# Pasqui1010/DART-Planner

Hardware: AMD Instinct MI355X
Metric: SE(3) rollouts/sec (N=30, batch=8192) + p95 solve ms, at 1/2/4/8 MI355X (higher is better)
Workload: dtype f32

## Files before the change

### dart_planner_amd/csrc/closed_loop_device.hpp

```cpp
#pragma once
#include <hip/hip_runtime.h>

#include <cmath>

#include "se3mpc_common.hpp"

static_assert(sizeof(se3mpc_controller_params) == 304, "se3mpc_controller_params is part of the C ABI (capi.py mirrors it)");
static_assert(sizeof(se3mpc_simulator_params) == 56, "se3mpc_simulator_params is part of the C ABI");

namespace se3mpc {

template <typename R>
struct CtrlDev {
  R kp_pos[3], ki_pos[3], kd_pos[3], kp_att[3], kd_att[3], inertia[3], max_torque[3], max_int_axis[3];
  R max_integral_pos, max_tilt, cos_max_tilt, gravity, max_thrust, min_thrust_abs, hover, track_thr, vel_thr, kb, decay, sat_thr,
      yaw_sing_thr, dh_cos, dh_sin;
  int anti_windup, fallback;
};

template <typename R>
static CtrlDev<R> make_ctrl_dev(const se3mpc_controller_params& p) {
  CtrlDev<R> c;
  for (int i = 0; i < 3; ++i) {
    c.kp_pos[i] = (R)p.kp_pos[i]; c.ki_pos[i] = (R)p.ki_pos[i]; c.kd_pos[i] = (R)p.kd_pos[i];
    c.kp_att[i] = (R)p.kp_att[i]; c.kd_att[i] = (R)p.kd_att[i]; c.inertia[i] = (R)p.inertia[i];
    c.max_torque[i] = (R)p.max_torque_xyz[i]; c.max_int_axis[i] = (R)p.max_integral_per_axis[i];
  }
  c.max_integral_pos = (R)p.max_integral_pos; c.max_tilt = (R)p.max_tilt_angle; c.cos_max_tilt = (R)std::cos(p.max_tilt_angle);
  c.gravity = (R)p.gravity; c.max_thrust = (R)p.max_thrust;
  c.min_thrust_abs = (R)(p.min_thrust * p.mass * p.gravity);
  c.hover = (R)(p.mass * p.gravity);
  c.track_thr = (R)p.tracking_error_threshold; c.vel_thr = (R)p.velocity_error_threshold;
  c.kb = (R)p.back_calculation_gain; c.decay = (R)p.integral_decay_factor; c.sat_thr = (R)p.saturation_threshold;
  c.yaw_sing_thr = (R)p.yaw_singularity_threshold;
  c.dh_cos = (R)std::cos(p.default_heading_yaw); c.dh_sin = (R)std::sin(p.default_heading_yaw);
  c.anti_windup = p.anti_windup_method; c.fallback = p.yaw_fallback_method;
  return c;
}

template <typename R>
struct SimDev {
  R mass, gravity, inertia[3], max_thrust, max_torque;
};
template <typename R>
static SimDev<R> make_sim_dev(const se3mpc_simulator_params& p) {
  SimDev<R> s;
  s.mass = (R)p.mass; s.gravity = (R)p.gravity; s.max_thrust = (R)p.max_thrust; s.max_torque = (R)p.max_torque;
  for (int i = 0; i < 3; ++i) s.inertia[i] = (R)p.inertia[i];
  return s;
}

template <typename R>
struct CtrlRegs {
  R integral[3];
  double last_time;
  R last_valid_thrust, unsat_thrust, unsat_torque[3];
  int failsafe_count, halvings, flags;
};

template <typename R>
__device__ __forceinline__ CtrlRegs<R> load_ctrl(const double* __restrict__ s) {
  CtrlRegs<R> r;
  for (int i = 0; i < 3; ++i) { r.integral[i] = (R)s[i]; r.unsat_torque[i] = (R)s[6 + i]; }
  r.last_time = s[3]; r.last_valid_thrust = (R)s[4]; r.unsat_thrust = (R)s[5];
  r.failsafe_count = (int)s[9]; r.halvings = (int)s[10]; r.flags = (int)s[11];
  return r;
}
template <typename R>
__device__ __forceinline__ void store_ctrl(double* __restrict__ s, const CtrlRegs<R>& r) {
  for (int i = 0; i < 3; ++i) { s[i] = (double)r.integral[i]; s[6 + i] = (double)r.unsat_torque[i]; }
  s[3] = r.last_time; s[4] = (double)r.last_valid_thrust; s[5] = (double)r.unsat_thrust;
  s[9] = (double)r.failsafe_count; s[10] = (double)r.halvings; s[11] = (double)r.flags;
}

template <typename R>
__device__ __forceinline__ R norm3(const R v[3]) { return sqrt(v[0] * v[0] + v[1] * v[1] + v[2] * v[2]); }
__device__ __forceinline__ void sin_cos(float x, float& s, float& c) { sincosf(x, &s, &c); }
__device__ __forceinline__ void sin_cos(double x, double& s, double& c) { sincos(x, &s, &c); }
template <typename R>
__device__ __forceinline__ R sign_of(R v) { return v > (R)0 ? (R)1 : (v < (R)0 ? (R)-1 : v); }
template <typename R>
__device__ __forceinline__ void cross3(const R a[3], const R b[3], R o[3]) {
  o[0] = a[1] * b[2] - a[2] * b[1]; o[1] = a[2] * b[0] - a[0] * b[2]; o[2] = a[0] * b[1] - a[1] * b[0];
}

template <typename R>
__device__ __forceinline__ void enter_failsafe(CtrlRegs<R>& s) {
  if (!(s.flags & 1)) {
    s.halvings += 1;
    s.integral[0] = s.integral[1] = s.integral[2] = (R)0;
    s.failsafe_count += 1;
  }
  s.flags |= 1;
}

enum { CF_FAILSAFE = 1, CF_BAD_DT = 2, CF_THRUST_SAT = 4, CF_SINGULAR = 8, CF_TILT = 16, CF_TORQUE_SAT_X = 32 };

template <typename R>
__device__ __forceinline__ void update_integral(const CtrlDev<R>& c, CtrlRegs<R>& s, const R ve[3], R dt, bool thrust_sat) {
  R upd[3];
  for (int i = 0; i < 3; ++i) upd[i] = ve[i] * dt;
  if (c.anti_windup == 0) {
    if (thrust_sat) for (int i = 0; i < 3; ++i) upd[i] = upd[i] * (R)0.1;
    for (int i = 0; i < 3; ++i) if (s.flags & (4 << i)) upd[i] = upd[i] * (R)0.1;
  } else if (c.anti_windup == 1) {
    if (thrust_sat) {
      const R fb = (s.unsat_thrust - c.max_thrust) * c.kb;
      upd[0] = upd[0] - fb * (R)0.33; upd[1] = upd[1] - fb * (R)0.33; upd[2] = upd[2] - fb * (R)0.34;
    }
    for (int i = 0; i < 3; ++i)
      if (s.flags & (4 << i)) upd[i] = upd[i] - ((s.unsat_torque[i] - c.max_torque[i]) * c.kb) * (R)0.5;
  }
  R I[3];
  for (int i = 0; i < 3; ++i) {
    I[i] = s.integral[i] + upd[i];
    if (fabs(I[i]) > c.max_int_axis[i]) I[i] = sign_of(I[i]) * c.max_int_axis[i];
  }
  const R mag = norm3(I);
  if (mag > c.max_integral_pos) { const R f = c.max_integral_pos / mag; for (int i = 0; i < 3; ++i) I[i] = I[i] * f; }
  for (int i = 0; i < 3; ++i) {
    if (fabs(I[i]) > c.max_int_axis[i] * c.sat_thr) I[i] = I[i] * c.decay;
    s.integral[i] = I[i];
  }
}

template <typename R>
__device__ __forceinline__ void desired_frame(const CtrlDev<R>& c, int method, bool force, const R yv[3], const R b3n[3], R cy, R sy, R b1[3],
                                              R b2[3], R& cos_angle, bool& singular) {
  cos_angle = fabs((yv[0] * b3n[0] + yv[1] * b3n[1]) + yv[2] * b3n[2]);
  singular = cos_angle >= c.yaw_sing_thr;
  if (singular || force) {
    R proj[3] = {(R)1 - b3n[0] * b3n[0], (R)0 - b3n[0] * b3n[1], (R)0 - b3n[0] * b3n[2]};
    const R np_ = norm3(proj);
    proj[0] = proj[0] / np_; proj[1] = proj[1] / np_; proj[2] = proj[2] / np_;
    if (method == 1 || method == 2) {
      const R hv[3] = {method == 1 ? c.dh_cos : cy, method == 1 ? c.dh_sin : sy, (R)0};
      R cx[3];
      cross3(hv, b3n, cx);
      const R nc = norm3(cx);
      if (nc > (R)1e-6) { b1[0] = cx[0] / nc; b1[1] = cx[1] / nc; b1[2] = cx[2] / nc; }
      else { b1[0] = proj[0]; b1[1] = proj[1]; b1[2] = proj[2]; }
    } else if (method != 0 || fabs(b3n[2]) < (R)0.99) {
      b1[0] = proj[0]; b1[1] = proj[1]; b1[2] = proj[2];
    } else {
      b1[0] = (R)1; b1[1] = (R)0; b1[2] = (R)0;
    }
  } else {
    cross3(yv, b3n, b1);
    const R n1 = norm3(b1);
    if (n1 > (R)1e-6) { b1[0] = b1[0] / n1; b1[1] = b1[1] / n1; b1[2] = b1[2] / n1; }
    else { b1[0] = (R)1; b1[1] = (R)0; b1[2] = (R)0; }
  }
  cross3(b3n, b1, b2);
}

template <typename R>
__device__ void attitude_torque(const CtrlDev<R>& c, CtrlRegs<R>& s, R scale, const R b3[3], const R att[3], const R omega[3], R yaw_des,
                                R yaw_rate_des, const R* Ifull, R torque_out[3], int& out_flags) {
  R cr, sr, cp, sp, cy, sy;
  sin_cos(att[0], sr, cr); sin_cos(att[1], sp, cp); sin_cos(att[2], sy, cy);
  const R Rm[3][3] = {{cy * cp, cy * sp * sr - sy * cr, cy * sp * cr + sy * sr},
                      {sy * cp, sy * sp * sr + cy * cr, sy * sp * cr - cy * sr},
                      {-sp, cp * sr, cp * cr}};
  R yc, ys;
  sin_cos(yaw_des, ys, yc);
  const R yv[3] = {yc, ys, (R)0};
  const R n3 = norm3(b3);
  const R b3n[3] = {b3[0] / n3, b3[1] / n3, b3[2] / n3};
  R b1[3], b2[3], cos_angle;
  bool singular;
  desired_frame(c, c.fallback, false, yv, b3n, cy, sy, b1, b2, cos_angle, singular);
  if (singular) out_flags |= CF_SINGULAR;
  const R Rd[3][3] = {{b1[0], b2[0], b3n[0]}, {b1[1], b2[1], b3n[1]}, {b1[2], b2[2], b3n[2]}};
  auto dtr = [&](const R A_[3][3], const R B_[3][3], int i, int j) { return (A_[0][i] * B_[0][j] + A_[1][i] * B_[1][j]) + A_[2][i] * B_[2][j]; };
  const R eR[3] = {(R)0.5 * (dtr(Rd, Rm, 2, 1) - dtr(Rm, Rd, 2, 1)), (R)0.5 * (dtr(Rd, Rm, 0, 2) - dtr(Rm, Rd, 0, 2)),
                   (R)0.5 * (dtr(Rd, Rm, 1, 0) - dtr(Rm, Rd, 1, 0))};
  const R eO[3] = {omega[0], omega[1], omega[2] - yaw_rate_des};
  R Iw[3];
  if (Ifull != nullptr) for (int i = 0; i < 3; ++i) Iw[i] = (Ifull[3 * i] * omega[0] + Ifull[3 * i + 1] * omega[1]) + Ifull[3 * i + 2] * omega[2];
  else for (int i = 0; i < 3; ++i) Iw[i] = c.inertia[i] * omega[i];
  R cor[3];
  cross3(omega, Iw, cor);
  int tsat = 0;
  for (int i = 0; i < 3; ++i) {
    R tq = (-(c.kp_att[i] * scale) * eR[i] - (c.kd_att[i] * scale) * eO[i]) + cor[i];
    s.unsat_torque[i] = tq;
    if (fabs(tq) > c.max_torque[i]) { tq = sign_of(tq) * c.max_torque[i]; tsat |= (4 << i); }
    torque_out[i] = tq;
  }
  s.flags = (s.flags & ~(4 | 8 | 16)) | tsat;
  out_flags |= (tsat >> 2) * CF_TORQUE_SAT_X;
}

template <typename R>
__device__ void attitude_command(const CtrlDev<R>& c, CtrlRegs<R>& s, R scale, const R tvw[3], R tm, const R att[3], const R omega[3],
                                 R yaw_des, R yaw_rate_des, R torque_out[3], int& out_flags) {
  R b3[3];
  if (tm > (R)1e-6) { b3[0] = tvw[0] / tm; b3[1] = tvw[1] / tm; b3[2] = tvw[2] / tm; }
  else { b3[0] = (R)0; b3[1] = (R)0; b3[2] = (R)1; }
  if (fmin(fmax(b3[2], (R)-1), (R)1) < c.cos_max_tilt) {
    const R sf = c.cos_max_tilt / b3[2];
    b3[0] = b3[0] * sf; b3[1] = b3[1] * sf; b3[2] = c.cos_max_tilt;
    const R n = norm3(b3);
    b3[0] = b3[0] / n; b3[1] = b3[1] / n; b3[2] = b3[2] / n;
    out_flags |= CF_TILT;
  }
  attitude_torque(c, s, scale, b3, att, omega, yaw_des, yaw_rate_des, (const R*)nullptr, torque_out, out_flags);
}

template <typename R>
__device__ void control_step(const CtrlDev<R>& c, CtrlRegs<R>& s, double t, const R pos[3], const R vel[3], const R att[3],
                             const R omega[3], const R dpos[3], const R dvel[3], const R dacc[3], R yaw_des, R yaw_rate_des,
                             R& thrust_out, R torque_out[3], int& out_flags) {
  out_flags = 0;
  const double dt_d = (s.last_time != s.last_time) ? 0.001 : t - s.last_time;
  s.last_time = t;
  if (dt_d <= 0.0 || dt_d > 0.1) {
    enter_failsafe(s);
    thrust_out = s.last_valid_thrust; torque_out[0] = torque_out[1] = torque_out[2] = (R)0;
    out_flags = CF_FAILSAFE | CF_BAD_DT;
    return;
  }
  const R dt = (R)dt_d;
  const R scale = (R)ldexp(1.0, -s.halvings);
  R pe[3], ve[3], tvw[3];
  for (int i = 0; i < 3; ++i) { pe[i] = dpos[i] - pos[i]; ve[i] = dvel[i] - vel[i]; }
  const R pen = norm3(pe), ven = norm3(ve);
  for (int i = 0; i < 3; ++i) {
    const R acc_pid = ((c.kp_pos[i] * scale) * pe[i] + (c.kd_pos[i] * scale) * ve[i]) + c.ki_pos[i] * s.integral[i];
    tvw[i] = dacc[i] + acc_pid;
  }
  tvw[2] = tvw[2] + c.gravity;
  R tm = norm3(tvw);
  s.unsat_thrust = tm;
  bool thrust_sat = false;
  if (tm > c.max_thrust) { tm = c.max_thrust; thrust_sat = true; }
  else if (tm < c.min_thrust_abs) { tm = c.min_thrust_abs; thrust_sat = true; }
  s.flags = (s.flags & ~2) | (thrust_sat ? 2 : 0);
  if (thrust_sat) out_flags |= CF_THRUST_SAT;
  update_integral(c, s, ve, dt, thrust_sat);
  if (pen > c.track_thr && ven > c.vel_thr) s.failsafe_count += 1;
  else s.failsafe_count = s.failsafe_count > 1 ? s.failsafe_count - 1 : 0;
  if (s.failsafe_count > 100) {
    enter_failsafe(s);
    thrust_out = s.last_valid_thrust; torque_out[0] = torque_out[1] = torque_out[2] = (R)0;
    out_flags |= CF_FAILSAFE;
    return;
  }
  attitude_command(c, s, scale, tvw, tm, att, omega, yaw_des, yaw_rate_des, torque_out, out_flags);
  s.last_valid_thrust = tm;
  s.flags &= ~1;
  s.failsafe_count = 0;
  thrust_out = tm;
}

template <typename R>
struct FastDev {
  R gravity, min_thrust_abs, hover;
};
template <typename R>
__device__ void control_step_fast(const CtrlDev<R>& c, const FastDev<R>& f, CtrlRegs<R>& s, double dt_d, const R pos[3], const R vel[3],
                                  const R att[3], const R omega[3], const R dpos[3], const R dvel[3], const R dacc[3], R yaw_des,
                                  R yaw_rate_des, R& thrust_out, R torque_out[3], int& out_flags) {
  out_flags = 0;
  if (dt_d <= 0.0 || dt_d > 0.1) {
    thrust_out = f.hover; torque_out[0] = torque_out[1] = torque_out[2] = (R)0;
    out_flags = CF_BAD_DT;
    return;
  }
  const R dt = (R)dt_d;
  const R scale = (R)ldexp(1.0, -s.halvings);
  R pe[3], ve[3], tvw[3];
  for (int i = 0; i < 3; ++i) { pe[i] = dpos[i] - pos[i]; ve[i] = dvel[i] - vel[i]; }
  for (int i = 0; i < 3; ++i) {
    const R acc_pid = ((c.kp_pos[i] * scale) * pe[i] + (c.kd_pos[i] * scale) * ve[i]) + c.ki_pos[i] * s.integral[i];
    tvw[i] = dacc[i] + acc_pid;
  }
  tvw[2] = tvw[2] + f.gravity;
  R tm = norm3(tvw);
  s.unsat_thrust = tm;
  bool thrust_sat = false;
  if (tm > c.max_thrust) { tm = c.max_thrust; thrust_sat = true; }
  else if (tm < f.min_thrust_abs) { tm = f.min_thrust_abs; thrust_sat = true; }
  s.flags = (s.flags & ~2) | (thrust_sat ? 2 : 0);
  if (thrust_sat) out_flags |= CF_THRUST_SAT;
  update_integral(c, s, ve, dt, thrust_sat);
  attitude_command(c, s, scale, tvw, tm, att, omega, yaw_des, yaw_rate_des, torque_out, out_flags);
  thrust_out = tm;
}

template <typename R>
struct PlanCursor {
  int idx;
  int rows_of;
  double t1, t2;
  R r1[9], r2[9];
};
template <typename R>
__device__ __forceinline__ void cursor_reset(PlanCursor<R>& c) { c.idx = 0; c.rows_of = -1; }

template <typename R>
__device__ __forceinline__ void sample_plan(double t, int N, const double* __restrict__ ts, const R* __restrict__ P, const R* __restrict__ V,
                                            const R* __restrict__ A, R tp[3], R tv[3], R ta[3], PlanCursor<R>& c) {
  int idx = c.idx;
  while (idx < N && ts[idx] < t) ++idx;
  c.idx = idx;
  if (idx != c.rows_of) {
    const int i1 = idx == 0 ? 0 : (idx >= N ? N - 1 : idx - 1), i2 = idx >= N ? N - 1 : idx;
    c.t1 = ts[i1]; c.t2 = ts[i2];
    for (int a = 0; a < 3; ++a) {
      c.r1[a] = P[3 * i1 + a]; c.r2[a] = P[3 * i2 + a];
      c.r1[3 + a] = V != nullptr ? V[3 * i1 + a] : (R)0; c.r2[3 + a] = V != nullptr ? V[3 * i2 + a] : (R)0;
      c.r1[6 + a] = A != nullptr ? A[3 * i1 + a] : (R)0; c.r2[6 + a] = A != nullptr ? A[3 * i2 + a] : (R)0;
    }
    c.rows_of = idx;
  }
  if (idx == 0 || idx >= N) {
    for (int a = 0; a < 3; ++a) { tp[a] = c.r1[a]; tv[a] = c.r1[3 + a]; ta[a] = c.r1[6 + a]; }
    return;
  }
  const R f = (R)((t - c.t1) / (c.t2 - c.t1));
  for (int a = 0; a < 3; ++a) {
    tp[a] = c.r1[a] + f * (c.r2[a] - c.r1[a]);
    tv[a] = c.r1[3 + a] + f * (c.r2[3 + a] - c.r1[3 + a]);
    ta[a] = c.r1[6 + a] + f * (c.r2[6 + a] - c.r1[6 + a]);
  }
}

template <typename R>
struct PlanView {
  int N;
  const double* ts; long long ts_stride;
  const R* P; long long sP;
  const R* V; long long sV;
  const R* A; long long sA;
  __device__ __forceinline__ PlanView of(int b) const {
    return {N, ts != nullptr ? ts + (size_t)b * ts_stride : nullptr, 0, P != nullptr ? P + (size_t)b * sP : nullptr, 0,
            V != nullptr ? V + (size_t)b * sV : nullptr, 0, A != nullptr ? A + (size_t)b * sA : nullptr, 0};
  }
};

template <typename R>
static inline bool plan_shape_ok(const PlanView<R>& p, int min_rows) {
  return p.N >= min_rows && p.N <= 4096 && p.ts_stride >= 0 && p.sP >= 0 && p.sV >= 0 && p.sA >= 0;
}
template <typename R>
static inline bool plan_present(const PlanView<R>& p) { return p.N <= 0 || (p.ts != nullptr && p.P != nullptr); }

template <typename R>
__device__ __forceinline__ void simulator_step(const SimDev<R>& m, R pos[3], R vel[3], R att[3], R omega[3], double& t, R thrust,
                                               const R torque[3], R dt, double dt_d, const R wind[3]) {
  thrust = fmin(fmax(thrust, (R)0), m.max_thrust);
  for (int i = 0; i < 3; ++i) {
    const R tq = fmin(fmax(torque[i], -m.max_torque), m.max_torque);
    const R wind_accel = wind[i] / m.mass;
    const R acc = ((i == 2 ? -m.gravity : (R)0) + (i == 2 ? thrust / m.mass : (R)0)) + wind_accel;
    vel[i] = vel[i] + acc * dt;
    pos[i] = pos[i] + vel[i] * dt;
    const R ang_acc = tq / m.inertia[i];
    omega[i] = omega[i] + ang_acc * dt;
    att[i] = att[i] + omega[i] * dt;
  }
  t = t + dt_d;
}

template <typename R>
__device__ __forceinline__ void cursor_before_step(PlanCursor<R>& cur, double sim_dt) {
  if (!(sim_dt > 0.0)) cur.idx = 0;
}

template <typename R>
__device__ __forceinline__ void flight_command(const CtrlDev<R>& c, CtrlRegs<R>& s, PlanCursor<R>& cur, int N, const double* ts, const R* P,
                                               const R* V, const R* A, const R p[3], const R v[3], const R a[3], const R w[3], double t,
                                               double sim_dt, R& th, R tq[3], R* target_row) {
  R tg[9];
  cursor_before_step(cur, sim_dt);
  sample_plan<R>(t, N, ts, P, V, A, tg, tg + 3, tg + 6, cur);
  if (target_row != nullptr) for (int i = 0; i < 9; ++i) target_row[i] = tg[i];
  int fl;
  control_step<R>(c, s, t, p, v, a, w, tg, tg + 3, tg + 6, (R)0, (R)0, th, tq, fl);
}

template <typename R>
__device__ __forceinline__ void flight_step(const CtrlDev<R>& c, const SimDev<R>& m, CtrlRegs<R>& s, PlanCursor<R>& cur, int N,
                                            const double* ts, const R* P, const R* V, const R* A, R p[3], R v[3], R a[3], R w[3], double& t,
                                            R dt, double sim_dt, const R wd[3], R& th, R tq[3]) {
  flight_command<R>(c, s, cur, N, ts, P, V, A, p, v, a, w, t, sim_dt, th, tq, (R*)nullptr);
  simulator_step<R>(m, p, v, a, w, t, th, tq, dt, sim_dt, wd);
}

template <typename R>
struct DroneBlock {
  double* stamps;
  double* time;
  double* ctrl;
  R *planP, *planV, *planA;
  R* vec;
};
template <typename R>
__device__ __forceinline__ DroneBlock<R> drone_block(unsigned char* base, int n, size_t plan_off, size_t vec_off) {
  DroneBlock<R> d;
  d.stamps = reinterpret_cast<double*>(base);
  d.time = d.stamps + n;
  d.ctrl = d.time + 1;
  d.planP = reinterpret_cast<R*>(base + plan_off);
  d.planV = d.planP + 3 * n;
  d.planA = d.planV + 3 * n;
  d.vec = reinterpret_cast<R*>(base + vec_off);
  return d;
}

template <typename R>
__device__ __forceinline__ void drone_load(const DroneBlock<R>& d, int b, const R* __restrict__ posg, const R* __restrict__ velg,
                                           const R* __restrict__ attg, const R* __restrict__ omegag, const R* __restrict__ windg,
                                           long long wind_stride, const double* __restrict__ timeg, const double* __restrict__ stateg) {
  for (int i = 0; i < 3; ++i) {
    d.vec[i] = posg[3 * b + i]; d.vec[3 + i] = velg[3 * b + i]; d.vec[6 + i] = attg[3 * b + i]; d.vec[9 + i] = omegag[3 * b + i];
    d.vec[12 + i] = windg != nullptr ? windg[(size_t)b * wind_stride + i] : (R)0;
  }
  *d.time = timeg[b];
  for (int i = 0; i < SE3MPC_CONTROLLER_STATE_WORDS; ++i) d.ctrl[i] = stateg[(size_t)b * SE3MPC_CONTROLLER_STATE_WORDS + i];
}
template <typename R>
__device__ __forceinline__ void drone_store(const DroneBlock<R>& d, int b, R* __restrict__ posg, R* __restrict__ velg, R* __restrict__ attg,
                                            R* __restrict__ omegag, double* __restrict__ timeg, double* __restrict__ stateg) {
  for (int i = 0; i < 3; ++i) { posg[3 * b + i] = d.vec[i]; velg[3 * b + i] = d.vec[3 + i]; attg[3 * b + i] = d.vec[6 + i]; omegag[3 * b + i] = d.vec[9 + i]; }
  timeg[b] = *d.time;
  for (int i = 0; i < SE3MPC_CONTROLLER_STATE_WORDS; ++i) stateg[(size_t)b * SE3MPC_CONTROLLER_STATE_WORDS + i] = d.ctrl[i];
}

template <typename IO>
__host__ __device__ constexpr size_t mc_plan_offset(int G) { return (size_t)(G + 1 + SE3MPC_CONTROLLER_STATE_WORDS) * sizeof(double); }
template <typename IO>
__host__ __device__ constexpr size_t mc_consts_offset(int G) { return (mc_plan_offset<IO>(G) + (size_t)(9 * G + 16) * sizeof(IO) + 15) / 16 * 16; }
template <typename IO>
__host__ __device__ constexpr size_t mc_group_bytes(int G) { return mc_consts_offset<IO>(G) + (sizeof(CtrlDev<IO>) + sizeof(SimDev<IO>) + 15) / 16 * 16; }

template <typename IO>
struct McBlock {
  DroneBlock<IO> d;
  CtrlDev<IO>* ctl;
  SimDev<IO>* sim;
};
template <typename IO, int G>
__device__ __forceinline__ McBlock<IO> mc_block(unsigned char* lds_raw, size_t solver_lds, int grp) {
  unsigned char* gb = lds_raw + solver_lds + (size_t)grp * mc_group_bytes<IO>(G);
  McBlock<IO> b;
  b.d = drone_block<IO>(gb, G, mc_plan_offset<IO>(G), mc_plan_offset<IO>(G) + (size_t)9 * G * sizeof(IO));
  b.ctl = reinterpret_cast<CtrlDev<IO>*>(gb + mc_consts_offset<IO>(G));
  b.sim = reinterpret_cast<SimDev<IO>*>(b.ctl + 1);
  return b;
}

#ifndef SE3MPC_MC_WAVES
#define SE3MPC_MC_WAVES 1
#endif

template <typename R>
struct DroneRegs {
  R p[3], v[3], a[3], w[3], wd[3];
  double t;
  __device__ __forceinline__ void load_state(int b, const R* __restrict__ pos, const R* __restrict__ vel, const R* __restrict__ att,
                                             const R* __restrict__ omega) {
    for (int i = 0; i < 3; ++i) { p[i] = pos[3 * b + i]; v[i] = vel[3 * b + i]; a[i] = att[3 * b + i]; w[i] = omega[3 * b + i]; }
  }
  __device__ __forceinline__ void load(int b, const R* __restrict__ pos, const R* __restrict__ vel, const R* __restrict__ att,
                                       const R* __restrict__ omega, const R* __restrict__ wind, long long wind_stride,
                                       const double* __restrict__ time) {
    load_state(b, pos, vel, att, omega);
    for (int i = 0; i < 3; ++i) wd[i] = wind != nullptr ? wind[(size_t)b * wind_stride + i] : (R)0;
    t = time[b];
  }
  __device__ __forceinline__ void store(int b, R* __restrict__ pos, R* __restrict__ vel, R* __restrict__ att, R* __restrict__ omega,
                                        double* __restrict__ time) const {
    for (int i = 0; i < 3; ++i) { pos[3 * b + i] = p[i]; vel[3 * b + i] = v[i]; att[3 * b + i] = a[i]; omega[3 * b + i] = w[i]; }
    time[b] = t;
  }
  __device__ __forceinline__ void load(const DroneBlock<R>& d) {
    for (int i = 0; i < 3; ++i) { p[i] = d.vec[i]; v[i] = d.vec[3 + i]; a[i] = d.vec[6 + i]; w[i] = d.vec[9 + i]; wd[i] = d.vec[12 + i]; }
    t = *d.time;
  }
  __device__ __forceinline__ void store(const DroneBlock<R>& d) const {
    for (int i = 0; i < 3; ++i) { d.vec[i] = p[i]; d.vec[3 + i] = v[i]; d.vec[6 + i] = a[i]; d.vec[9 + i] = w[i]; }
    *d.time = t;
  }
};

template <typename R, typename F>
__device__ __forceinline__ void fly_steps(const CtrlDev<R> c, const SimDev<R> m, const DroneBlock<R>& d, int N, int n, double sim_dt,
                                          F&& after_step) {
  CtrlRegs<R> s = load_ctrl<R>(d.ctrl);
  DroneRegs<R> r;
  r.load(d);
  const R dt = (R)sim_dt;
  PlanCursor<R> cur;
  cursor_reset(cur);
  for (int step = 0; step < n; ++step) {
    R th, tq[3];
    flight_step<R>(c, m, s, cur, N, d.stamps, d.planP, d.planV, d.planA, r.p, r.v, r.a, r.w, r.t, dt, sim_dt, r.wd, th, tq);
    after_step(step, r.p);
  }
  r.store(d);
  store_ctrl<R>(d.ctrl, s);
}

template <typename R, typename F>
__device__ __forceinline__ int lane_loop(DroneRegs<R>& d, int b, int B, int nsteps, int gust_step, R gx, R gy, R gz, bool stop_at_plan_end,
                                         double ts_last, R* __restrict__ log_state, R* __restrict__ log_cmd, double* __restrict__ log_time,
                                         F&& fly) {
  int taken = 0;
  bool active = true;
  for (int step = 0; step < nsteps; ++step) {
    if (stop_at_plan_end && d.t > ts_last) active = false;
    if (log_state != nullptr) {
      R* ls = log_state + ((size_t)step * B + b) * 12;
      for (int i = 0; i < 3; ++i) { ls[i] = d.p[i]; ls[3 + i] = d.v[i]; ls[6 + i] = d.a[i]; ls[9 + i] = d.w[i]; }
    }
    if (log_time != nullptr) log_time[(size_t)step * B + b] = d.t;
    R th = (R)NAN, tq[3] = {(R)NAN, (R)NAN, (R)NAN};
    if (active) {
      if (step == gust_step) { d.wd[0] = gx; d.wd[1] = gy; d.wd[2] = gz; }
      fly(step, th, tq);
      ++taken;
    }
    if (log_cmd != nullptr) {
      R* lc = log_cmd + ((size_t)step * B + b) * 4;
      lc[0] = th; lc[1] = tq[0]; lc[2] = tq[1]; lc[3] = tq[2];
    }
  }
  return taken;
}

static inline int check_controller_params(const se3mpc_controller_params* p) {
  if (p == nullptr) return SE3MPC_ERR_NULL;
  const double* d = reinterpret_cast<const double*>(p);
  for (int i = 0; i < 37; ++i)
    if (!std::isfinite(d[i])) return SE3MPC_ERR_PARAM;
  if (!(p->mass > 0.0) || p->anti_windup_method < 0 || p->anti_windup_method > 2 || p->yaw_fallback_method < 0 || p->yaw_fallback_method > 3)
    return SE3MPC_ERR_PARAM;
  return SE3MPC_OK;
}

static inline int check_simulator_params(const se3mpc_simulator_params* sp) {
  if (sp == nullptr) return SE3MPC_ERR_NULL;
  if (!(sp->mass > 0.0) || !std::isfinite(sp->gravity) || !(sp->inertia[0] > 0.0) || !(sp->inertia[1] > 0.0) || !(sp->inertia[2] > 0.0) ||
      !std::isfinite(sp->max_thrust) || !std::isfinite(sp->max_torque))
    return SE3MPC_ERR_PARAM;
  return SE3MPC_OK;
}

__device__ __forceinline__ double plan_stamp(int cycle, int substeps, double sim_dt, int k, double dt) {
  const double base = (double)(cycle * substeps) * sim_dt;
  const double off = (double)k * dt;
  return base + off;
}

}
```

### dart_planner_amd/csrc/monte_carlo.hip

```cpp
#include "solve_device.hpp"
#pragma clang fp contract(off)
#include "closed_loop_device.hpp"
#pragma clang fp contract(fast)

namespace se3mpc {

template <typename IO, int G>
__global__ void __launch_bounds__(64, SE3MPC_MC_WAVES)
monte_carlo_kernel(SolveDev q, CtrlDev<IO> ctl, SimDev<IO> sim, int B, int cycles, int substeps, double sim_dt, size_t solver_lds,
                   const IO* __restrict__ goalg, const IO* __restrict__ windg, long long wind_stride, double* __restrict__ timeg,
                   IO* __restrict__ posg, IO* __restrict__ velg, IO* __restrict__ attg, IO* __restrict__ omegag,
                   double* __restrict__ stateg, IO* __restrict__ Xg, IO* __restrict__ accg, se3mpc_solve_info* __restrict__ infog,
                   int* __restrict__ overflowed) {
  HIP_DYNAMIC_SHARED(unsigned char, lds_raw)
  constexpr int P = kWave / G, J = kSlots;
  const int lane = lane_id();
  const int k = lane & (G - 1);
  const int grp = lane / G;
  const int pb = blockIdx.x * P + grp;
  if (pb >= B) return;
  double goal[3] = {0.0, 0.0, 0.0};
  if (q.has_goal) {
#pragma unroll
    for (int a = 0; a < 3; ++a) goal[a] = (double)goalg[pb * 3 + a];
  }
  if (k == 0) {
    const McBlock<IO> blk = mc_block<IO, G>(lds_raw, solver_lds, grp);
    *blk.ctl = ctl; *blk.sim = sim;
    drone_load<IO>(blk.d, pb, posg, velg, attg, omegag, windg, wind_stride, timeg, stateg);
  }
  group_sync<G>();
  const IO* x0row = nullptr;
  const bool cold = true;
  for (int cycle = 0; cycle < cycles; ++cycle) {
    double ps[3], vs[3];
    {
      const IO* s_vec = mc_block<IO, G>(lds_raw, solver_lds, grp).d.vec;
#pragma unroll
      for (int a = 0; a < 3; ++a) { ps[a] = (double)s_vec[a]; vs[a] = (double)s_vec[3 + a]; }
    }
    double x[J];
    {
#include "solve_body.inc"
      if (task == SE3MPC_TASK_OVERFLOW && k == 0) atomicAdd(overflowed, 1);
      const DroneBlock<IO> drone = mc_block<IO, G>(lds_raw, solver_lds, grp).d;
      if (live) {
#pragma unroll
        for (int a = 0; a < 3; ++a) { drone.planP[3 * k + a] = (IO)x[a]; drone.planV[3 * k + a] = (IO)x[3 + a]; }
        drone.planA[3 * k + 0] = (IO)(x[6] / q.mass); drone.planA[3 * k + 1] = (IO)(x[7] / q.mass); drone.planA[3 * k + 2] = (IO)(x[8] / q.mass - q.grav);
        drone.stamps[k] = plan_stamp(cycle, substeps, sim_dt, k, q.dt);
      }
      if (cycle == cycles - 1 && live) {
        if (Xg != nullptr) {
#pragma unroll
          for (int j = 0; j < J; ++j) Xg[(size_t)pb * n + (j / 3) * n3 + 3 * k + (j % 3)] = (IO)x[j];
        }
        if (accg != nullptr) {
          const size_t o = (size_t)pb * n3 + 3 * k;
          accg[o] = drone.planA[3 * k + 0]; accg[o + 1] = drone.planA[3 * k + 1]; accg[o + 2] = drone.planA[3 * k + 2];
        }
        if (infog != nullptr && k == 0) {
          se3mpc_solve_info r;
          r.fun = f; r.nit = nit; r.nfev = nfev; r.status = status; r.task = task;
          infog[pb] = r;
        }
      }
    }
    group_sync<G>();
    if (k == 0) {
      const McBlock<IO> blk = mc_block<IO, G>(lds_raw, solver_lds, grp);
      const CtrlDev<IO> c = *blk.ctl;
      const SimDev<IO> m = *blk.sim;
      fly_steps<IO>(c, m, blk.d, q.N, substeps, sim_dt, [](int, const IO*) {});
    }
    group_sync<G>();
  }
  if (k == 0) drone_store<IO>(mc_block<IO, G>(lds_raw, solver_lds, grp).d, pb, posg, velg, attg, omegag, timeg, stateg);
}

template <typename IO>
int monte_carlo_impl(const se3mpc_params* p, const se3mpc_controller_params* cp, const se3mpc_simulator_params* sp, int B, int cycles,
                     int substeps, double sim_dt, const IO* goal, const IO* wind, long long wind_stride, double* time, IO* pos, IO* vel,
                     IO* att, IO* omega, double* state, IO* X_last, IO* acc_last, se3mpc_solve_info* info_last, int32_t* overflowed,
                     void* stream) {
  if (p == nullptr || cp == nullptr || sp == nullptr) return SE3MPC_ERR_NULL;
  int rc = check_params_impl(p);
  if (rc) return rc;
  rc = check_controller_params(cp);
  if (rc) return rc;
  rc = check_simulator_params(sp);
  if (rc) return rc;
  if (B < 0 || cycles < 0 || substeps < 0 || p->horizon > kWave) return SE3MPC_ERR_SHAPE;
  if (!std::isfinite(sim_dt)) return SE3MPC_ERR_PARAM;
  if (wind != nullptr && !(wind_stride == 0 || wind_stride >= 3)) return SE3MPC_ERR_SHAPE;
  if (B == 0) return SE3MPC_OK;
  if (!time || !pos || !vel || !att || !omega || !state || !overflowed || (p->has_goal && !goal)) return SE3MPC_ERR_NULL;
  hipStream_t s = (hipStream_t)stream;
  if (hipMemsetAsync(overflowed, 0, sizeof(int32_t), s) != hipSuccess) return launch_status("se3mpc_monte_carlo(memset)");
  SolveDev q = make_solve_dev(*p);
  const int G = solve_group_for_horizon(p->horizon);
  const int waves = (int)(((long)B * G + kWave - 1) / kWave);
  const size_t extra = (size_t)(kWave / G) * mc_group_bytes<IO>(G);
  const size_t per_cu = (size_t)(waves + 255) / 256;
  const size_t budget = (size_t)160 * 1024 / (per_cu < 1 ? 1 : (per_cu > 8 ? 8 : per_cu));
  int mlds = q.m;
  while (mlds > 4 && solve_lds_bytes(mlds, G, sizeof(IO)) + extra > budget) --mlds;
  q.mlds = mlds;
  const size_t solver_lds = (solve_lds_bytes(mlds, G, sizeof(IO)) + 15) / 16 * 16;
  const size_t lds = solver_lds + extra;
  const CtrlDev<IO> c = make_ctrl_dev<IO>(*cp);
  const SimDev<IO> m = make_sim_dev<IO>(*sp);
  dispatch_group(G, [&](auto g) {
    constexpr int GG = decltype(g)::value;
    if (lds > 64 * 1024)
      (void)hipFuncSetAttribute(reinterpret_cast<const void*>(&monte_carlo_kernel<IO, GG>), hipFuncAttributeMaxDynamicSharedMemorySize, (int)lds);
    hipLaunchKernelGGL((monte_carlo_kernel<IO, GG>), dim3(waves), dim3(kWave), lds, s, q, c, m, B, cycles, substeps, sim_dt, solver_lds, goal,
                       wind, wind_stride, time, pos, vel, att, omega, state, X_last, acc_last, info_last, overflowed);
  });
  return launch_status("se3mpc_monte_carlo");
}

}

using namespace se3mpc;

extern "C" int se3mpc_monte_carlo_f32(const se3mpc_params* p, const se3mpc_controller_params* cp, const se3mpc_simulator_params* sp, int B,
                                      int cycles, int substeps, double sim_dt, const float* goal, const float* wind, long long wind_stride,
                                      double* time, float* pos, float* vel, float* att, float* omega, double* state, float* X_last,
                                      float* acc_last, se3mpc_solve_info* info_last, int32_t* overflowed, void* stream) {
  return monte_carlo_impl<float>(p, cp, sp, B, cycles, substeps, sim_dt, goal, wind, wind_stride, time, pos, vel, att, omega, state, X_last,
                                 acc_last, info_last, overflowed, stream);
}
extern "C" int se3mpc_monte_carlo_f64(const se3mpc_params* p, const se3mpc_controller_params* cp, const se3mpc_simulator_params* sp, int B,
                                      int cycles, int substeps, double sim_dt, const double* goal, const double* wind, long long wind_stride,
                                      double* time, double* pos, double* vel, double* att, double* omega, double* state, double* X_last,
                                      double* acc_last, se3mpc_solve_info* info_last, int32_t* overflowed, void* stream) {
  return monte_carlo_impl<double>(p, cp, sp, B, cycles, substeps, sim_dt, goal, wind, wind_stride, time, pos, vel, att, omega, state, X_last,
                                  acc_last, info_last, overflowed, stream);
}
```

Before: 8.056 billion.

## Fly drone substeps with whole solver group, splitting sin/cos across lanes

Previously only lane 0 of each solver group ran the closed-loop flight substeps while the other lanes idled. Now every lane of the group runs the flight steps redundantly, and the four sin/cos evaluations in the attitude controller are spread across lanes 0..3 and broadcast back with group shuffles. Lane 0 still writes the state back to memory. This removes divergence-serialised transcendental work, at the cost of extra cross-lane broadcasts and redundant arithmetic on every lane.

```diff
diff --git a/dart_planner_amd/csrc/closed_loop_device.hpp b/dart_planner_amd/csrc/closed_loop_device.hpp
--- a/dart_planner_amd/csrc/closed_loop_device.hpp
+++ b/dart_planner_amd/csrc/closed_loop_device.hpp
@@ -4,6 +4,7 @@
 #include <cmath>
 
 #include "se3mpc_common.hpp"
+#include <se3mpc_wave_ops.hpp>
 
 static_assert(sizeof(se3mpc_controller_params) == 304, "se3mpc_controller_params is part of the C ABI (capi.py mirrors it)");
 static_assert(sizeof(se3mpc_simulator_params) == 56, "se3mpc_simulator_params is part of the C ABI");
@@ -77,6 +78,29 @@
 __device__ __forceinline__ R norm3(const R v[3]) { return sqrt(v[0] * v[0] + v[1] * v[1] + v[2] * v[2]); }
 __device__ __forceinline__ void sin_cos(float x, float& s, float& c) { sincosf(x, &s, &c); }
 __device__ __forceinline__ void sin_cos(double x, double& s, double& c) { sincos(x, &s, &c); }
+
+struct SoloLanes {
+  template <typename R>
+  __device__ __forceinline__ static void sin_cos4(const R x[4], R s[4], R c[4]) {
+    sin_cos(x[0], s[0], c[0]); sin_cos(x[1], s[1], c[1]); sin_cos(x[2], s[2], c[2]); sin_cos(x[3], s[3], c[3]);
+  }
+};
+template <int G>
+struct TeamLanes {
+  __device__ __forceinline__ static float bcast(float v, int src) { return __int_as_float(group_bcast<G>(__float_as_int(v), src)); }
+  __device__ __forceinline__ static double bcast(double v, int src) { return group_bcast<G>(v, src); }
+  template <typename R>
+  __device__ __forceinline__ static void sin_cos4(const R x[4], R s[4], R c[4]) {
+    static_assert(G >= 8, "lanes 0..3 of a group");
+    const int i = lane_id() & 3;
+    const R mine = i == 0 ? x[0] : (i == 1 ? x[1] : (i == 2 ? x[2] : x[3]));
+    R sm, cm;
+    sin_cos(mine, sm, cm);
+#pragma unroll
+    for (int j = 0; j < 4; ++j) { s[j] = bcast(sm, j); c[j] = bcast(cm, j); }
+  }
+};
+
 template <typename R>
 __device__ __forceinline__ R sign_of(R v) { return v > (R)0 ? (R)1 : (v < (R)0 ? (R)-1 : v); }
 template <typename R>
@@ -154,16 +178,16 @@
   cross3(b3n, b1, b2);
 }
 
-template <typename R>
+template <typename R, typename T = SoloLanes>
 __device__ void attitude_torque(const CtrlDev<R>& c, CtrlRegs<R>& s, R scale, const R b3[3], const R att[3], const R omega[3], R yaw_des,
                                 R yaw_rate_des, const R* Ifull, R torque_out[3], int& out_flags) {
-  R cr, sr, cp, sp, cy, sy;
-  sin_cos(att[0], sr, cr); sin_cos(att[1], sp, cp); sin_cos(att[2], sy, cy);
+  const R ang[4] = {att[0], att[1], att[2], yaw_des};
+  R sn[4], cs[4];
+  T::sin_cos4(ang, sn, cs);
+  const R sr = sn[0], cr = cs[0], sp = sn[1], cp = cs[1], sy = sn[2], cy = cs[2], ys = sn[3], yc = cs[3];
   const R Rm[3][3] = {{cy * cp, cy * sp * sr - sy * cr, cy * sp * cr + sy * sr},
                       {sy * cp, sy * sp * sr + cy * cr, sy * sp * cr - cy * sr},
                       {-sp, cp * sr, cp * cr}};
-  R yc, ys;
-  sin_cos(yaw_des, ys, yc);
   const R yv[3] = {yc, ys, (R)0};
   const R n3 = norm3(b3);
   const R b3n[3] = {b3[0] / n3, b3[1] / n3, b3[2] / n3};
@@ -192,7 +216,7 @@
   out_flags |= (tsat >> 2) * CF_TORQUE_SAT_X;
 }
 
-template <typename R>
+template <typename R, typename T = SoloLanes>
 __device__ void attitude_command(const CtrlDev<R>& c, CtrlRegs<R>& s, R scale, const R tvw[3], R tm, const R att[3], const R omega[3],
                                  R yaw_des, R yaw_rate_des, R torque_out[3], int& out_flags) {
   R b3[3];
@@ -205,10 +229,10 @@
     b3[0] = b3[0] / n; b3[1] = b3[1] / n; b3[2] = b3[2] / n;
     out_flags |= CF_TILT;
   }
-  attitude_torque(c, s, scale, b3, att, omega, yaw_des, yaw_rate_des, (const R*)nullptr, torque_out, out_flags);
-}
-
-template <typename R>
+  attitude_torque<R, T>(c, s, scale, b3, att, omega, yaw_des, yaw_rate_des, (const R*)nullptr, torque_out, out_flags);
+}
+
+template <typename R, typename T = SoloLanes>
 __device__ void control_step(const CtrlDev<R>& c, CtrlRegs<R>& s, double t, const R pos[3], const R vel[3], const R att[3],
                              const R omega[3], const R dpos[3], const R dvel[3], const R dacc[3], R yaw_des, R yaw_rate_des,
                              R& thrust_out, R torque_out[3], int& out_flags) {
@@ -247,7 +271,7 @@
     out_flags |= CF_FAILSAFE;
     return;
   }
-  attitude_command(c, s, scale, tvw, tm, att, omega, yaw_des, yaw_rate_des, torque_out, out_flags);
+  attitude_command<R, T>(c, s, scale, tvw, tm, att, omega, yaw_des, yaw_rate_des, torque_out, out_flags);
   s.last_valid_thrust = tm;
   s.flags &= ~1;
   s.failsafe_count = 0;
@@ -369,7 +393,7 @@
   if (!(sim_dt > 0.0)) cur.idx = 0;
 }
 
-template <typename R>
+template <typename R, typename T = SoloLanes>
 __device__ __forceinline__ void flight_command(const CtrlDev<R>& c, CtrlRegs<R>& s, PlanCursor<R>& cur, int N, const double* ts, const R* P,
                                                const R* V, const R* A, const R p[3], const R v[3], const R a[3], const R w[3], double t,
                                                double sim_dt, R& th, R tq[3], R* target_row) {
@@ -378,14 +402,14 @@
   sample_plan<R>(t, N, ts, P, V, A, tg, tg + 3, tg + 6, cur);
   if (target_row != nullptr) for (int i = 0; i < 9; ++i) target_row[i] = tg[i];
   int fl;
-  control_step<R>(c, s, t, p, v, a, w, tg, tg + 3, tg + 6, (R)0, (R)0, th, tq, fl);
-}
-
-template <typename R>
+  control_step<R, T>(c, s, t, p, v, a, w, tg, tg + 3, tg + 6, (R)0, (R)0, th, tq, fl);
+}
+
+template <typename R, typename T = SoloLanes>
 __device__ __forceinline__ void flight_step(const CtrlDev<R>& c, const SimDev<R>& m, CtrlRegs<R>& s, PlanCursor<R>& cur, int N,
                                             const double* ts, const R* P, const R* V, const R* A, R p[3], R v[3], R a[3], R w[3], double& t,
                                             R dt, double sim_dt, const R wd[3], R& th, R tq[3]) {
-  flight_command<R>(c, s, cur, N, ts, P, V, A, p, v, a, w, t, sim_dt, th, tq, (R*)nullptr);
+  flight_command<R, T>(c, s, cur, N, ts, P, V, A, p, v, a, w, t, sim_dt, th, tq, (R*)nullptr);
   simulator_step<R>(m, p, v, a, w, t, th, tq, dt, sim_dt, wd);
 }
 
@@ -502,6 +526,27 @@
   }
   r.store(d);
   store_ctrl<R>(d.ctrl, s);
+}
+
+template <int G, typename R, typename F>
+__device__ __forceinline__ void fly_steps_team(const CtrlDev<R> c, const SimDev<R> m, const DroneBlock<R>& d, int k, int N, int n,
+                                               double sim_dt, F&& after_step) {
+  CtrlRegs<R> s = load_ctrl<R>(d.ctrl);
+  DroneRegs<R> r;
+  r.load(d);
+  const R dt = (R)sim_dt;
+  PlanCursor<R> cur;
+  cursor_reset(cur);
+  for (int step = 0; step < n; ++step) {
+    R th, tq[3];
+    flight_step<R, TeamLanes<G>>(c, m, s, cur, N, d.stamps, d.planP, d.planV, d.planA, r.p, r.v, r.a, r.w, r.t, dt, sim_dt, r.wd, th, tq);
+    after_step(step, r.p);
+  }
+  group_sync<G>();
+  if (k == 0) {
+    r.store(d);
+    store_ctrl<R>(d.ctrl, s);
+  }
 }
 
 template <typename R, typename F>
diff --git a/dart_planner_amd/csrc/monte_carlo.hip b/dart_planner_amd/csrc/monte_carlo.hip
--- a/dart_planner_amd/csrc/monte_carlo.hip
+++ b/dart_planner_amd/csrc/monte_carlo.hip
@@ -67,11 +67,11 @@
       }
     }
     group_sync<G>();
-    if (k == 0) {
+    {
       const McBlock<IO> blk = mc_block<IO, G>(lds_raw, solver_lds, grp);
       const CtrlDev<IO> c = *blk.ctl;
       const SimDev<IO> m = *blk.sim;
-      fly_steps<IO>(c, m, blk.d, q.N, substeps, sim_dt, [](int, const IO*) {});
+      fly_steps_team<G, IO>(c, m, blk.d, k, q.N, substeps, sim_dt, [](int, const IO*) {});
     }
     group_sync<G>();
   }
```

After: 8.073 billion, median of 5. No clear change (+0.2%).
